# mcveanlab/Corticall

Measured on AMD Instinct MI355X. Metric: k-mers traversed/sec (whole node) + contigs/sec, k=47 3-color LdBG, higher is better.
Workload: dtype u64

## Files before the change

corticall_amd/csrc/capi.cpp:

```cpp
#include <string.h>

#include <memory>

#include "build.h"
#include "cursor.h"
#include "engine_host.h"
#include "linkbuild.h"
#include "mosaic.h"
#include "seeds.h"
#include "select.h"
#include "shard.h"
#include "sw.h"
#include "thread.h"
#include "unitigs.h"
#include "variants.h"

using namespace ldbg;

namespace ldbg {
int64_t sort_ctx_file(const std::string& in_path, const std::string& out_path, int device);
int64_t subset_ctx_file(const std::string& in_path, const int64_t* indices, int64_t n, const std::string& out_path);
int64_t join_ctx_files(const std::vector<std::string>& paths, const std::string& out_path, int device);
std::vector<uint8_t> join_ctx_image(const std::vector<std::string>& paths, int device, bool find_view);
void profile_reset_all();
// ... 786 lines not shown
}
ldbg_status ldbg_cursor_result_get(const ldbg_cursor_result* r, int64_t* offsets, uint64_t* kmer_words, int64_t* rec, int32_t* n_reverse, int32_t* n_forward,
                                   int64_t* seed_rec, uint8_t* end_reverse, uint8_t* end_forward, uint8_t* status) {
    return guard([&] { cursor_result_of(r).get(offsets, kmer_words, rec, n_reverse, n_forward, seed_rec, end_reverse, end_forward, status, false, nullptr); });
}
ldbg_status ldbg_cursor_result_get_dev(const ldbg_cursor_result* r, void* d_offsets, void* d_kmer_words, void* d_rec, void* d_n_reverse, void* d_n_forward,
                                       void* d_seed_rec, void* d_end_reverse, void* d_end_forward, void* d_status, void* stream) {
    return guard([&] {
        cursor_result_of(r).get(d_offsets, d_kmer_words, d_rec, d_n_reverse, d_n_forward, d_seed_rec, d_end_reverse, d_end_forward, d_status, true, (rt::stream_t)stream);
    });
}
ldbg_status ldbg_cursor_result_free(ldbg_cursor_result* r) { delete r; return LDBG_OK; }

static ldbg_status variant_batch_any(ldbg_engine* ce, ldbg_engine* pe, const char* seeds, int64_t n, bool on_device, int stop_colour, int64_t max_steps, uint64_t sum_mask,
                                     ldbg_variant_result** out) {
    return guard([&] {
        if (!ce || !pe || !out) throw StatusError(LDBG_ERR_ARG, "variant batch: null engine or result pointer");
        *out = nullptr;
        if (!ce->cursor_batch) ce->cursor_batch.reset(new CursorBatchHost(ce->e));
        if (!pe->cursor_batch) pe->cursor_batch.reset(new CursorBatchHost(pe->e));
        std::unique_ptr<VariantResult> r(variant_batch(ce->e, *ce->cursor_batch, pe->e, *pe->cursor_batch, seeds, n, on_device, stop_colour, max_steps, sum_mask));
        *out = new ldbg_variant_result{std::move(r)};
    });
}
ldbg_status ldbg_engine_variant_batch(ldbg_engine* child_engine, ldbg_engine* parent_engine, const char* seeds, int64_t n, int stop_colour, int64_t max_steps,
                                      uint64_t sum_mask, ldbg_variant_result** out) {
    return variant_batch_any(child_engine, parent_engine, seeds, n, false, stop_colour, max_steps, sum_mask, out);
}
ldbg_status ldbg_engine_variant_batch_device(ldbg_engine* child_engine, ldbg_engine* parent_engine, const void* d_seeds, int64_t n, int stop_colour, int64_t max_steps,
                                             uint64_t sum_mask, ldbg_variant_result** out) {
    return variant_batch_any(child_engine, parent_engine, (const char*)d_seeds, n, true, stop_colour, max_steps, sum_mask, out);
}
static const VariantResult& variant_result_of(const ldbg_variant_result* r) {
    if (!r || !r->r) throw StatusError(LDBG_ERR_ARG, "no variant result");
    return *r->r;
}
ldbg_status ldbg_variant_result_sizes(const ldbg_variant_result* r, int64_t* n_seeds, int* n_colours, int64_t* allele_bytes, int64_t* n_child_vertices,
                                      int64_t* n_parent_vertices, int* kmer_words) {
    return guard([&] {
        const VariantResult& v = variant_result_of(r);
        if (n_seeds) *n_seeds = v.n;
        if (n_colours) *n_colours = v.n_colours;
        if (allele_bytes) *allele_bytes = v.allele_bytes;
        if (n_child_vertices) *n_child_vertices = v.child ? v.child->total : 0;
        if (n_parent_vertices) *n_parent_vertices = v.parent ? v.parent->total : 0;
        if (kmer_words) *kmer_words = v.W;
    });
}
ldbg_status ldbg_variant_result_get(const ldbg_variant_result* r, const ldbg_variant_arrays* into) {
    return guard([&] {
        if (!into) throw StatusError(LDBG_ERR_ARG, "variant result: null arrays");
        variant_result_of(r).get(*into, false, nullptr);
    });
}
ldbg_status ldbg_variant_result_get_dev(const ldbg_variant_result* r, const ldbg_variant_arrays* into, void* stream) {
    return guard([&] {
        if (!into) throw StatusError(LDBG_ERR_ARG, "variant result: null arrays");
        variant_result_of(r).get(*into, true, (rt::stream_t)stream);
    });
}
ldbg_status ldbg_variant_result_free(ldbg_variant_result* r) { delete r; return LDBG_OK; }

ldbg_status ldbg_mosaic_align_batch(int device, const ldbg_mosaic_params* p, int64_t n, const char* queries, const int64_t* query_off, const int64_t* target_first,
                                    const char* targets, const int64_t* target_off, ldbg_mosaic_result** out) {
    return guard([&] {
        if (!out) throw StatusError(LDBG_ERR_ARG, "mosaic: null result pointer");
        *out = nullptr;
        if (!p) throw StatusError(LDBG_ERR_ARG, "mosaic: null parameters");
        std::unique_ptr<MosaicResult> r(mosaic_align_batch(device, *p, n, queries, query_off, target_first, targets, target_off));
        *out = new ldbg_mosaic_result{std::move(r)};
    });
}
static const MosaicResult& mosaic_result_of(const ldbg_mosaic_result* r) {
    if (!r || !r->r) throw StatusError(LDBG_ERR_ARG, "no mosaic result");
    return *r->r;
}
ldbg_status ldbg_mosaic_result_sizes(const ldbg_mosaic_result* r, int64_t* n, int64_t* path_entries) {
    return guard([&] {
        const MosaicResult& m = mosaic_result_of(r);
        if (n) *n = m.n;
        if (path_entries) *path_entries = m.path_off.back();
    });
}
ldbg_status ldbg_mosaic_result_get(const ldbg_mosaic_result* r, const ldbg_mosaic_arrays* into) {
    return guard([&] {
        if (!into) throw StatusError(LDBG_ERR_ARG, "mosaic result: null arrays");
        const MosaicResult& m = mosaic_result_of(r);
        auto copy = [](void* dst, const void* src, size_t bytes) { if (dst && bytes) memcpy(dst, src, bytes); };
        copy(into->status, m.status.data(), m.status.size());
        copy(into->llk, m.llk.data(), m.llk.size() * 8);
        copy(into->path_off, m.path_off.data(), m.path_off.size() * 8);
        copy(into->copy, m.copy.data(), m.copy.size() * 4);
        copy(into->state, m.state.data(), m.state.size() * 4);
        copy(into->pos, m.pos.data(), m.pos.size() * 4);
    });
}
ldbg_status ldbg_mosaic_result_free(ldbg_mosaic_result* r) { delete r; return LDBG_OK; }
ldbg_status ldbg_mosaic_tb_roundtrip(int device, double div, int64_t n, const int32_t* who, const int32_t* state, const int32_t* pos, int32_t* out) {
    return guard([&] { mosaic_tb_roundtrip(device, div, n, who, state, pos, out); });
}

ldbg_status ldbg_sw_align_batch(int device, int64_t n, const char* queries, const int64_t* query_off, const char* subjects, const int64_t* subject_off,
                                ldbg_sw_result** out) {
    return guard([&] {
        if (!out) throw StatusError(LDBG_ERR_ARG, "sw: null result pointer");
        *out = nullptr;
        std::unique_ptr<SwResult> r(sw_align_batch(device, n, queries, query_off, subjects, subject_off));
        *out = new ldbg_sw_result{std::move(r)};
    });
}
static const SwResult& sw_result_of(const ldbg_sw_result* r) {
    if (!r || !r->r) throw StatusError(LDBG_ERR_ARG, "no sw result");
    return *r->r;
}
ldbg_status ldbg_sw_result_sizes(const ldbg_sw_result* r, int64_t* n, int64_t* columns, int64_t* query_letters, int64_t* subject_letters) {
    return guard([&] {
        const SwResult& m = sw_result_of(r);
        if (n) *n = m.n;
        if (columns) *columns = m.col_off.back();
        if (query_letters) *query_letters = m.q_off.back();
        if (subject_letters) *subject_letters = m.s_off.back();
    });
}
ldbg_status ldbg_sw_result_get(const ldbg_sw_result* r, const ldbg_sw_arrays* into) {
    return guard([&] {
        if (!into) throw StatusError(LDBG_ERR_ARG, "sw result: null arrays");
        const SwResult& m = sw_result_of(r);
        auto copy = [](void* dst, const void* src, size_t bytes) { if (dst && bytes) memcpy(dst, src, bytes); };
        copy(into->status, m.status.data(), m.status.size());
        copy(into->score, m.score.data(), m.score.size() * 8);
        copy(into->end_q, m.end_q.data(), m.end_q.size() * 4);
        copy(into->end_s, m.end_s.data(), m.end_s.size() * 4);
        copy(into->begin_q, m.begin_q.data(), m.begin_q.size() * 4);
        copy(into->begin_s, m.begin_s.data(), m.begin_s.size() * 4);
        copy(into->aligned_len, m.aligned_len.data(), m.aligned_len.size() * 4);
        copy(into->edits, m.edits.data(), m.edits.size() * 4);
        copy(into->col_off, m.col_off.data(), m.col_off.size() * 8);
        copy(into->cols, m.cols.data(), m.cols.size());
        copy(into->q_off, m.q_off.data(), m.q_off.size() * 8);
        copy(into->q_letters, m.q_letters.data(), m.q_letters.size());
        copy(into->s_off, m.s_off.data(), m.s_off.size() * 8);
        copy(into->s_letters, m.s_letters.data(), m.s_letters.size());
    });
}
ldbg_status ldbg_sw_result_free(ldbg_sw_result* r) { delete r; return LDBG_OK; }

#ifdef LDBG_HOSTSIM
void ldbg_debug_ls(uint64_t* out) {
    auto& d = ldbg::ls_debug();
    out[0] = d.adds; out[1] = d.newkeys; out[2] = d.choices; out[3] = d.scan; out[4] = d.maxn; out[5] = d.steps; out[6] = d.sum_n;
    out[7] = d.runs_a; out[8] = d.runs_b; out[9] = d.run_vertices; out[10] = d.retries; out[11] = d.repeats;
    d = ldbg::LsDebug();
}
#endif
#ifdef LDBG_HOSTSIM
extern "C" void ldbg_hostsim_set_lanes(int n) { int v = 1; while (v * 2 <= n && v < 64) v *= 2; ::ldbg::sim::lanes_setting() = v; }
#endif
ldbg_status ldbg_profile_reset(void) { profile_reset_all(); return LDBG_OK; }
ldbg_status ldbg_profile_get(const char* family, double* total_ms, int64_t* launches) {
    profile_get(family, total_ms, launches);
    return LDBG_OK;
}

}
```

corticall_amd/csrc/engine.h:

```cpp
#pragma once
#include "graph.h"
#include "links.h"

namespace ldbg {

struct RunIndexView { const uint64_t* uinfo; const uint32_t* uo; const uint8_t* ubase; };

struct EngineView {
    GraphView g;
    uint32_t trav_mask, recruit_mask, join_mask;
    uint32_t trav_sel4, recruit_sel4;
    int first_trav;
    int stopper, max_len, connect_all, strict_flip;
    int lean_rows;
    int cursor_on;
    uint32_t link_flag_mask;
    LinksView links;
    RunIndexView runs;
};

enum : uint32_t {
    ST_OK = 0,
    ST_NULLPTR = 1,
    ST_LINKSTORE_FULL = 2,
    ST_BRANCH_NULL = 3,
    ST_COPY_OVERFLOW = 4,
    ST_POOL_FULL = 5,
    ST_STOPPER_CONFIG = 6,
    ST_DEPTH_OVERFLOW = 7,
    ST_TABLE_FULL = 8,
    ST_LOG_FULL = 9,
    ST_RETRY_PLAIN = 10,
    ST_MERGE_UNSUPPORTED = 11
};

LDBG_HOSTDEV uint64_t path_pack(int64_t idx, bool flip, unsigned base, int copy, bool quirk = false) {
    return (uint64_t)(idx + 1) | ((uint64_t)(flip ? 1 : 0) << 33) | ((uint64_t)(base & 3u) << 34) |
           (((uint64_t)(uint32_t)copy & 0xFFFFFFull) << 36) | ((uint64_t)(quirk ? 1 : 0) << 60);
}
LDBG_HOSTDEV bool path_quirk(uint64_t e) { return (e >> 60) & 1ull; }
LDBG_HOSTDEV int64_t path_idx(uint64_t e) { return (int64_t)(e & 0x1FFFFFFFFull) - 1; }
LDBG_HOSTDEV bool path_flip(uint64_t e) { return (e >> 33) & 1ull; }
LDBG_HOSTDEV unsigned path_base(uint64_t e) { return (unsigned)((e >> 34) & 3ull); }
LDBG_HOSTDEV int path_copy(uint64_t e) { int32_t v = (int32_t)((e >> 36) & 0xFFFFFFull); return (v << 8) >> 8; }

LDBG_HOSTDEV int popc4(uint32_t m) { return (int)((m & 1u) + ((m >> 1) & 1u) + ((m >> 2) & 1u) + ((m >> 3) & 1u)); }
LDBG_HOSTDEV unsigned lowbit4(uint32_t m) { return (m & 1u) ? 0u : ((m & 2u) ? 1u : ((m & 4u) ? 2u : 3u)); }

struct Node {
    int32_t idx;
    int32_t copy;
    uint32_t vslot;
    uint64_t vent;
    uint8_t flip;
    uint8_t fj;
    uint8_t npe;
    uint8_t lflags;
    uint8_t next_mask;
    uint8_t prev_mask;
    uint8_t base;
    uint8_t e1;
#ifdef LDBG_LEAN_PROFILE
    unsigned long long p1, p2;
#endif
    uint32_t ent1;
    uint64_t ui;
};

template <bool FEW = false>
LDBG_HOSTDEV void node_fill_bytes(const EngineView& e, Node& n, uint32_t edges4, const uint8_t* more, uint8_t fl) {
    const GraphView& g = e.g;
    n.npe = 0; n.fj = n.flip;
    n.lflags = fl & LDBG_ROW_LINK_BITS;
    if (e.strict_flip && (fl & LDBG_ROW_HASH_COLLISION)) n.fj = 0;
    const bool fj = n.fj != 0;
    uint32_t tb = edges4 & e.trav_sel4, rb = edges4 & e.recruit_sel4;
    tb |= tb >> 16; tb |= tb >> 8; rb |= rb >> 16; rb |= rb >> 8;
    if (!FEW)
        for (int col = 4; col < g.C; col++) {
            if ((e.trav_mask >> col) & 1u) tb |= more[col];
            if ((e.recruit_mask >> col) & 1u) rb |= more[col];
        }
    tb &= 0xffu; rb &= 0xffu;
    const uint32_t tfw = !fj ? tb & 0xf : tb >> 4, trn = !fj ? tb >> 4 : tb & 0xf;
    const uint32_t rfw = !fj ? rb & 0xf : rb >> 4, rrn = !fj ? rb >> 4 : rb & 0xf;
    const uint32_t tf = tfw, rf = rfw;
    const uint32_t tr = ((trn & 1u) << 3) | ((trn & 2u) << 1) | ((trn & 4u) >> 1) | ((trn & 8u) >> 3);
    const uint32_t rr = ((rrn & 1u) << 3) | ((rrn & 2u) << 1) | ((rrn & 4u) >> 1) | ((rrn & 8u) >> 3);
    n.next_mask = (uint8_t)(tf ? tf : rf);
    n.prev_mask = (uint8_t)(tr ? tr : rr);
}
LDBG_HOSTDEV void node_fill(const EngineView& e, Node& n) {
    const GraphView& g = e.g;
    n.ui = e.runs.uinfo && n.idx >= 0 ? e.runs.uinfo[n.idx] : 0ull;
    if (n.idx >= 0) {
        const uint8_t* row = graph_row(g, n.idx);
        const uint8_t* ed = row + g.edges_off;
        uint32_t edges4 = 0;
        for (int col = 0; col < g.C && col < 4; col++) edges4 |= (uint32_t)ed[col] << (8 * col);
        node_fill_bytes(e, n, edges4, ed, row[g.flags_off]);
    } else {
        n.npe = e.recruit_mask != 0 ? 1 : 0; n.lflags = 0; n.fj = n.flip;
        n.next_mask = n.prev_mask = 0;
    }
}

LDBG_HOSTDEV void node_child(const EngineView& e, const Node& p, bool fwd, unsigned base, Node& n) {
    const GraphView& g = e.g;
    const bool fj = p.fj != 0;
    const unsigned j = fwd ? (!fj ? base : 4u + (3u - base)) : (!fj ? 4u + base : (3u - base));
    const uint32_t ent = graph_nbr(g, p.idx, (int)j);
    n.idx = (int32_t)(ent & 0x7FFFFFFFu) - 1;
    n.copy = 0; n.vslot = 0; n.vent = 0; n.base = (uint8_t)base; n.e1 = 0; n.ent1 = 0;
    bool flip = (((ent >> 31) & 1u) != 0) != fj;
    if (n.idx >= 0 && (graph_row(g, n.idx)[g.flags_off] & LDBG_ROW_PALINDROME)) flip = false;
    n.flip = flip ? 1 : 0;
    node_fill(e, n);
}

template <int W>
LDBG_HOSTDEV Kmer<W> node_kmer(const EngineView& e, const Node& n) {
    Kmer<W> c = graph_key<W>(e.g, n.idx);
    return n.flip ? kmer_revcomp<W>(c, e.g.k) : c;
}
template <int W>
LDBG_HOSTDEV Kmer<W> node_o(const EngineView& e, const Node& n) {
    Kmer<W> c = graph_key<W>(e.g, n.idx);
    return n.fj ? kmer_revcomp<W>(c, e.g.k) : c;
}
template <int W>
LDBG_HOSTDEV Kmer<W> child_kmer(const EngineView& e, const Node& p, bool fwd, unsigned base) {
    Kmer<W> o = node_o<W>(e, p);
    return fwd ? kmer_next<W>(o, e.g.k, base) : kmer_prev<W>(o, e.g.k, base);
}
template <int W>
LDBG_HOSTDEV void node_find(const EngineView& e, const Kmer<W>& sk, Node& n) {
    bool fc;
    Kmer<W> c = kmer_canonical<W>(sk, e.g.k, &fc);
    n.idx = (int32_t)graph_find_canonical<W>(e.g, c);
    n.copy = 0; n.vslot = 0; n.vent = 0; n.base = 0; n.e1 = 0; n.ent1 = 0;
    n.flip = fc ? 1 : 0;
    node_fill(e, n);
    if (n.idx < 0 && e.strict_flip && fc)
        n.fj = kmer_java_hash<W>(c, e.g.k) != kmer_java_hash<W>(sk, e.g.k) ? 1 : 0;
}
LDBG_HOSTDEV void node_null(const EngineView& e, Node& n) {
    n.idx = -1; n.copy = 0; n.vslot = 0; n.vent = 0; n.e1 = 0; n.ent1 = 0; n.flip = 0; n.fj = 0; n.lflags = 0; n.base = 0;
    n.next_mask = n.prev_mask = 0; n.ui = 0;
    n.npe = e.recruit_mask != 0 ? 1 : 0;
}

struct VisitedTable {
    uint64_t* tab;
    uint32_t mask;
    uint32_t used;
};
#define LDBG_VT_KEY_MASK 0x3FFFFFFFFull
LDBG_HOSTDEV uint32_t vt_hash(uint64_t key) {
    uint32_t x = (uint32_t)key ^ ((uint32_t)(key >> 32) * 0x9E3779B1u);
    x ^= x >> 16; x *= 0x85EBCA6Bu; x ^= x >> 13; x *= 0xC2B2AE35u; x ^= x >> 16;
    return x;
}
LDBG_HOSTDEV uint64_t vt_key(int64_t idx, bool flip) { return ((uint64_t)(idx + 1) << 1) | (flip ? 1ull : 0ull); }
#ifdef LDBG_HOSTSIM
struct LsDebug { uint64_t adds = 0, newkeys = 0, choices = 0, scan = 0, maxn = 0, steps = 0, sum_n = 0, runs_a = 0, runs_b = 0, run_vertices = 0, retries = 0, repeats = 0; };
inline LsDebug& ls_debug() { static LsDebug d; return d; }
#endif
struct VtPeek { uint64_t e[4]; };
LDBG_HOSTDEV VtPeek vt_peek(const VisitedTable& t, uint32_t h) {
    VtPeek p;
#pragma unroll
    for (uint32_t q = 0; q < 4; q++) p.e[q] = LDBG_GLOBAL(const uint64_t, t.tab)[(h + q) & t.mask];
    return p;
}
LDBG_HOSTDEV uint32_t vt_probe_from(VisitedTable& t, uint64_t key, uint32_t h, VtPeek pk, uint64_t* ent) {
    while (true) {
#ifdef LDBG_HOSTSIM
        ls_debug().scan++;
#endif
        uint32_t q = 4;
        uint64_t ev = 0;
#pragma unroll
        for (int i = 3; i >= 0; i--) {
            const bool stop = pk.e[i] == 0 || (pk.e[i] & LDBG_VT_KEY_MASK) == key;
            q = stop ? (uint32_t)i : q;
            ev = stop ? pk.e[i] : ev;
        }
        if (q < 4) {
            const uint32_t slot = (h + q) & t.mask;
            if (ev == 0) { LDBG_GLOBAL(uint64_t, t.tab)[slot] = key; t.used++; ev = key; }
            *ent = ev;
            return slot;
        }
        h = (h + 4) & t.mask;
        pk = vt_peek(t, h);
    }
}
LDBG_HOSTDEV uint32_t vt_locate(VisitedTable& t, int64_t idx, bool flip, uint64_t* ent) {
    const uint64_t key = vt_key(idx, flip);
    const uint32_t h = vt_hash(key) & t.mask;
    return vt_probe_from(t, key, h, vt_peek(t, h), ent);
}
LDBG_HOSTDEV int vt_count_e(uint64_t e) { return (int)((e >> 48) & 0x7FFFull); }
#define LDBG_VT_EPOCH_MAX 0x3FFFu
LDBG_HOSTDEV bool vt_seen_e(uint64_t e, uint32_t epoch) { return (uint32_t)((e >> 34) & LDBG_VT_EPOCH_MAX) == epoch; }
LDBG_HOSTDEV uint64_t vt_with_seen(uint64_t e, uint32_t epoch) { return (e & ~((uint64_t)LDBG_VT_EPOCH_MAX << 34)) | ((uint64_t)epoch << 34); }
LDBG_HOSTDEV uint64_t vt_with_count(uint64_t e, int c) { return (e & ~(0x7FFFull << 48)) | ((uint64_t)(c & 0x7FFF) << 48); }
LDBG_HOSTDEV void node_locate(VisitedTable& t, Node& n) { if (n.idx >= 0) n.vslot = vt_locate(t, n.idx, n.flip != 0, &n.vent); }
LDBG_HOSTDEV int node_count(const Node& n) { return n.idx >= 0 ? vt_count_e(n.vent) : 0; }
LDBG_HOSTDEV void node_store(VisitedTable& t, Node& n, uint64_t val) { LDBG_GLOBAL(uint64_t, t.tab)[n.vslot] = val; n.vent = val; }
LDBG_HOSTDEV void node_sync(Node& n, const Node& written) { if (n.idx >= 0 && written.idx >= 0 && n.vslot == written.vslot) n.vent = written.vent; }
LDBG_HOSTDEV uint32_t node_child_entry(const EngineView& e, const Node& p, bool fwd, unsigned base) {
    const bool fj = p.fj != 0;
    const unsigned j = fwd ? (!fj ? base : 4u + (3u - base)) : (!fj ? 4u + base : (3u - base));
    return graph_nbr(e.g, p.idx, (int)j);
}
LDBG_HOSTDEV unsigned nbr_slot(bool fj, bool fwd, unsigned base) {
    return fwd ? (!fj ? base : 4u + (3u - base)) : (!fj ? 4u + base : (3u - base));
}
LDBG_HOSTDEV uint32_t nbr_pick(const uint32_t (&nb)[8], unsigned j) {
    uint32_t v = reg_opaque(nb[0]);
#pragma unroll
    for (unsigned q = 1; q < 8; q++) v = j == q ? reg_opaque(nb[q]) : v;
    return v;
}
LDBG_HOSTDEV bool row_is_packed(const GraphView& g) { return g.C <= 3 && (g.edges_off & 3) == 0 && (g.nbr_off & 15) == 0 && (g.stride & 15) == 0; }
LDBG_HOSTDEV constexpr bool row_layout_is_packed(int W, int C) {
    return C <= 3 && (row_layout(W, C).edges_off & 3) == 0 && (row_layout(W, C).nbr_off & 15) == 0 && (row_layout(W, C).stride & 15) == 0;
}
template <bool LEAN = false>
LDBG_HOSTDEV void node_from_entry(const EngineView& e, VisitedTable& t, const Node& p, uint32_t ent, unsigned base, bool fwd, Node& n) {
    const GraphView& g = e.g;
    const bool fj = p.fj != 0;
    n.idx = (int32_t)(ent & 0x7FFFFFFFu) - 1;
    n.copy = 0; n.vslot = 0; n.vent = 0; n.base = (uint8_t)base; n.e1 = 0; n.ent1 = 0;
    bool flip = (((ent >> 31) & 1u) != 0) != fj;
    const bool rec = LEAN || n.idx >= 0;
    const bool early = LEAN || (rec && (g.k & 1));
    uint64_t key = 0;
    VtPeek e0 = {{0, 0, 0, 0}};
    uint32_t h = 0;
    if (early) { key = vt_key(n.idx, flip); h = vt_hash(key) & t.mask; e0 = vt_peek(t, h); }
    uint32_t nb[8] = {0, 0, 0, 0, 0, 0, 0, 0};
    uint32_t ef = 0;
    const bool packed = LEAN || row_is_packed(g);
    uint64_t ui = 0;
    if (rec && e.runs.uinfo) ui = LDBG_GLOBAL(const uint64_t, e.runs.uinfo)[n.idx];
    if (rec) {
        const uint8_t* row = graph_row(g, n.idx);
        if (packed) {
            struct alignas(16) U4 { uint32_t x, y, z, w; };
            const U4 a = *(const U4*)(row + g.nbr_off), b = *(const U4*)(row + g.nbr_off + 16);
            ef = *(const uint32_t*)(row + g.edges_off);
            nb[0] = a.x; nb[1] = a.y; nb[2] = a.z; nb[3] = a.w; nb[4] = b.x; nb[5] = b.y; nb[6] = b.z; nb[7] = b.w;
        } else {
            const uint32_t* nbp = (const uint32_t*)(row + g.nbr_off);
#pragma unroll
            for (int q = 0; q < 8; q++) nb[q] = nbp[q];
        }
    }
    if (!LEAN && rec && !(g.k & 1) && (graph_row(g, n.idx)[g.flags_off] & LDBG_ROW_PALINDROME)) flip = false;
#ifdef LDBG_LEAN_PROFILE
    if (LEAN) {
        asm volatile("" ::: "memory");
        const unsigned long long t1 = __builtin_readcyclecounter();
        asm volatile("s_waitcnt vmcnt(0)" ::: "memory");
        const unsigned long long t2 = __builtin_readcyclecounter();
        n.p1 = t1; n.p2 = t2;
    }
#endif
    n.flip = flip ? 1 : 0;
    if (LEAN) node_fill_bytes<true>(e, n, ef & ((1u << (8 * g.C)) - 1u), nullptr, (uint8_t)(ef >> (8 * g.C)));
    else if (rec && packed) node_fill_bytes(e, n, ef & ((1u << (8 * g.C)) - 1u), nullptr, (uint8_t)(ef >> (8 * g.C)));
    else node_fill(e, n);
    n.ui = ui;
    if (rec) {
        const uint32_t m = fwd ? n.next_mask : n.prev_mask;
        const unsigned j = nbr_slot(n.fj != 0, fwd, lowbit4(m));
        const uint32_t v = nbr_pick(nb, j);
        const bool one = popc4(m) == 1;
        n.ent1 = one ? v : 0u; n.e1 = one ? 1 : 0;
        if (!early) { key = vt_key(n.idx, flip); h = vt_hash(key) & t.mask; e0 = vt_peek(t, h); }
        n.vslot = vt_probe_from(t, key, h, e0, &n.vent);
    }
}
struct NodeLoad {
    uint32_t nb[8];
    uint32_t ef, h;
    uint64_t ui, key;
    VtPeek e0;
    int32_t idx;
    bool flip;
};
LDBG_HOSTDEV void node_issue_lean(const EngineView& e, const VisitedTable& t, bool parent_fj, uint32_t ent, NodeLoad& L) {
    const GraphView& g = e.g;
    L.idx = (int32_t)(ent & 0x7FFFFFFFu) - 1;
    L.flip = (((ent >> 31) & 1u) != 0) != parent_fj;
    L.key = vt_key(L.idx, L.flip);
    L.h = vt_hash(L.key) & t.mask;
    L.e0 = vt_peek(t, L.h);
    L.ui = e.runs.uinfo ? LDBG_GLOBAL(const uint64_t, e.runs.uinfo)[L.idx] : 0ull;
    const uint8_t* row = graph_row(g, L.idx);
    struct alignas(16) U4 { uint32_t x, y, z, w; };
    const U4 a = *(const U4*)(row + g.nbr_off), b = *(const U4*)(row + g.nbr_off + 16);
    L.ef = *(const uint32_t*)(row + g.edges_off);
    L.nb[0] = a.x; L.nb[1] = a.y; L.nb[2] = a.z; L.nb[3] = a.w; L.nb[4] = b.x; L.nb[5] = b.y; L.nb[6] = b.z; L.nb[7] = b.w;
}
LDBG_HOSTDEV bool vt_round_covers(const VisitedTable& t, uint32_t h, uint32_t slot) { return slot != 0xFFFFFFFFu && ((slot - h) & t.mask) < 4u; }
LDBG_HOSTDEV void node_finish_lean(const EngineView& e, VisitedTable& t, const NodeLoad& L, unsigned base, bool fwd, Node& n, uint32_t claimed0 = 0xFFFFFFFFu,
                                   uint32_t claimed1 = 0xFFFFFFFFu) {
    const GraphView& g = e.g;
    n.idx = L.idx;
    n.copy = 0; n.vslot = 0; n.vent = 0; n.base = (uint8_t)base; n.e1 = 0; n.ent1 = 0;
    n.flip = L.flip ? 1 : 0;
    node_fill_bytes<true>(e, n, L.ef & ((1u << (8 * g.C)) - 1u), nullptr, (uint8_t)(L.ef >> (8 * g.C)));
    n.ui = L.ui;
    const uint32_t m = fwd ? n.next_mask : n.prev_mask;
    const unsigned j = nbr_slot(n.fj != 0, fwd, lowbit4(m));
    const uint32_t v = nbr_pick(L.nb, j);
    const bool one = popc4(m) == 1;
    n.ent1 = one ? v : 0u; n.e1 = one ? 1 : 0;
    const bool stale = vt_round_covers(t, L.h, claimed0) || vt_round_covers(t, L.h, claimed1);
    n.vslot = vt_probe_from(t, L.key, L.h, stale ? vt_peek(t, L.h) : L.e0, &n.vent);
}
LDBG_HOSTDEV void node_child_located(const EngineView& e, VisitedTable& t, const Node& p, bool fwd, unsigned base, Node& n) {
    node_from_entry(e, t, p, node_child_entry(e, p, fwd, base), base, fwd, n);
}

struct LsElem {
    uint32_t str_off;
    uint32_t birth;
    int32_t hash;
    uint32_t key_seq;
    uint16_t len;
    uint16_t pos;
    uint8_t comp;
    uint8_t nxn;
    uint16_t nx;
};
static_assert(sizeof(LsElem) == 24, "LsElem is moved as six words");
#ifdef LDBG_HOSTSIM
struct LdsShadow { const char* base = nullptr; size_t bytes = 0; std::vector<uint8_t> written; bool on = false; };
inline LdsShadow& lds_shadow() { static LdsShadow s; return s; }
inline void lds_shadow_begin(const void* base, size_t bytes) {
    LdsShadow& s = lds_shadow();
    static const bool want = getenv("LDBG_HOSTSIM_LDS_CHECK") != nullptr;
    s.on = want;
    if (!want) return;
    s.base = (const char*)base; s.bytes = bytes; s.written.assign(bytes / 24 + 1, 0);
}
inline void lds_shadow_touch(const void* q, bool write) {
    LdsShadow& s = lds_shadow();
    if (!s.on || (const char*)q < s.base || (const char*)q >= s.base + s.bytes) return;
    const size_t i = (size_t)((const char*)q - s.base) / 24;
    if (write) { s.written[i] = 1; return; }
    if (!s.written[i]) {
        fprintf(stderr, "[hostsim] link-store element %zu of the simulated LDS is read before this wavefront wrote it\n", i);
        void* bt[48]; const int nb = backtrace(bt, 48); backtrace_symbols_fd(bt, nb, 2);
        abort();
    }
}
#endif
template <typename P> LDBG_HOSTDEV LsElem ls_elem_in(P q) {
#ifdef LDBG_HOSTSIM
    lds_shadow_touch((const void*)q, false);
#endif
    uint32_t w[6];
#pragma unroll
    for (int i = 0; i < 6; i++) w[i] = q[i];
    LsElem x;
    __builtin_memcpy(&x, w, 24);
    return x;
}
template <typename P> LDBG_HOSTDEV void ls_elem_out(P q, const LsElem& x) {
#ifdef LDBG_HOSTSIM
    lds_shadow_touch((const void*)q, true);
#endif
    uint32_t w[6];
    __builtin_memcpy(w, &x, 24);
#pragma unroll
    for (int i = 0; i < 6; i++) q[i] = w[i];
}
#ifdef LDBG_HOSTSIM
inline uint32_t& ls_peak_elements() { static uint32_t p = 0; return p; }
#define LDBG_LS_PEAK(i) do { if ((uint32_t)(i) + 1u > ::ldbg::ls_peak_elements()) ::ldbg::ls_peak_elements() = (uint32_t)(i) + 1u; } while (0)
#else
#define LDBG_LS_PEAK(i) ((void)0)
#endif
#if defined(LDBG_WALK_DIAG) && defined(__HIP_DEVICE_COMPILE__)
#define LDBG_LS_COUNT(ctr, tail) do { if (ctr) { atomicAdd((ctr), 1ull); if (tail) atomicAdd((ctr) + 1, 1ull); } } while (0)
#else
#define LDBG_LS_COUNT(ctr, tail) ((void)0)
#endif
struct LinkStoreDev {
#ifdef LDBG_WALK_DIAG
    unsigned long long* diag;
#endif
    LsElem* fast;
    LsElem* el;
    uint32_t fast_cap, fast_stride;
    uint32_t cap;
    uint32_t n;
    uint32_t java_cap;
    uint32_t nkeys;
    uint32_t next_seq;
    uint32_t age;
    uint32_t n_new;
    bool overflow;
};
LDBG_HOSTDEV LsElem ls_get(const LinkStoreDev& s, uint32_t i) {
    LDBG_LS_COUNT(s.diag, i >= s.fast_cap);
    if (i < s.fast_cap) return ls_elem_in(LDBG_LDS(const uint32_t, s.fast + i * s.fast_stride));
    return ls_elem_in(LDBG_GLOBAL(const uint32_t, s.el + (i - s.fast_cap)));
}
LDBG_HOSTDEV void ls_set(LinkStoreDev& s, uint32_t i, const LsElem& x) {
    LDBG_LS_COUNT(s.diag, i >= s.fast_cap);
    LDBG_LS_PEAK(i);
    if (i < s.fast_cap) ls_elem_out(LDBG_LDS(uint32_t, s.fast + i * s.fast_stride), x);
    else ls_elem_out(LDBG_GLOBAL(uint32_t, s.el + (i - s.fast_cap)), x);
}
LDBG_HOSTDEV void ls_clear(LinkStoreDev& s) { s.n = 0; s.java_cap = 0; s.nkeys = 0; s.next_seq = 0; s.age = 0; s.n_new = 0; s.overflow = false; }
struct LsSaved { uint32_t n, java_cap, nkeys, next_seq, age, n_new; uint8_t overflow; };
LDBG_HOSTDEV LsSaved ls_save(const LinkStoreDev& s) { return LsSaved{s.n, s.java_cap, s.nkeys, s.next_seq, s.age, s.n_new, (uint8_t)(s.overflow ? 1 : 0)}; }
LDBG_HOSTDEV void ls_restore(LinkStoreDev& s, const LsSaved& v) {
    s.n = v.n; s.java_cap = v.java_cap; s.nkeys = v.nkeys; s.next_seq = v.next_seq; s.age = v.age; s.n_new = v.n_new; s.overflow = v.overflow != 0;
}
struct LsWave {
#ifdef LDBG_WALK_DIAG
    unsigned long long* diag;
#endif
    LsElem* fast;
    uint32_t stride;
    uint32_t fast_cap;
    LsElem* el;
    uint32_t ecap;
};
LDBG_HOSTDEV unsigned ls_char(const LinksView& L, const LsElem& x, uint32_t i) {
    unsigned b = L.bases[x.str_off + i];
    return x.comp ? 3u - b : b;
}
LDBG_HOSTDEV void ls_fill_nx(const LinksView& L, LsElem& x) {
    uint32_t nx = 0, cnt = 0;
    for (uint32_t i = 0; i < 8; i++) {
        if ((uint32_t)x.pos + i >= x.len) break;
        nx |= (uint32_t)ls_char(L, x, (uint32_t)x.pos + i) << (2 * i);
        cnt++;
    }
    x.nx = (uint16_t)nx; x.nxn = (uint8_t)cnt;
}
LDBG_HOSTDEV void ls_first_nx(const JuncRec& jr, LsElem& x) {
    const uint32_t cnt = jr.len < 8u ? jr.len : 8u;
    const uint32_t mask = (1u << (2 * cnt)) - 1u;
    const uint32_t nx = jr.is_fw >> 16;
    x.nx = (uint16_t)((x.comp ? ~nx : nx) & mask);
    x.nxn = (uint8_t)cnt;
}
LDBG_HOSTDEV unsigned ls_cur(const LsElem& x) { return x.nx & 3u; }
LDBG_HOSTDEV void ls_advance(const LinksView& L, LsElem& x) {
    x.pos++;
    x.nx >>= 2; x.nxn--;
    if (x.nxn == 0) ls_fill_nx(L, x);
}
LDBG_HOSTDEV bool ls_same_string(const LinksView& L, const LsElem& a, const LsElem& b) {
    if (a.str_off == b.str_off && a.comp == b.comp) return true;
    if (a.len != b.len || a.hash != b.hash) return false;
    for (uint32_t i = 0; i < a.len; i++) if (ls_char(L, a, i) != ls_char(L, b, i)) return false;
    return true;
}
LDBG_HOSTDEV bool ls_key_alive(const LinkStoreDev& s, uint32_t key_seq, uint32_t n) {
    for (uint32_t i = n; i-- > 0;) if (ls_get(s, i).key_seq == key_seq) return true;
    return false;
}
LDBG_HOSTDEV void ls_add(const LinksView& L, LinkStoreDev& s, uint32_t jlo, uint32_t jhi, bool query_flipped, bool fwd) {
    for (uint32_t j = jlo; j < jhi; j++) {
        const JuncRec jr = L.junc[j];
        bool lgf = ((jr.is_fw & 1u) != 0) != query_flipped;
// ... 184 lines not shown
```

corticall_amd/csrc/runstep.h:

```cpp
#pragma once
#include "lscoop.h"
#include "runs.h"
#include "strand.h"

namespace ldbg {

#define LDBG_RUN_MIN 8u

struct Piece {
    uint32_t S, E;
    uint32_t q, n;
    bool plus, asc;
};
LDBG_DEV void piece_cut(uint32_t& S, uint32_t& E, uint32_t pos, uint32_t cut) {
    if (cut >= S && cut <= E) {
        if (pos < cut) E = cut - 1u;
        else if (pos > cut) S = cut + 1u;
        else S = E = pos;
    }
}
LDBG_DEV Piece piece_make(uint64_t ui, bool flip, bool fwd, uint32_t S, uint32_t E) {
    Piece p;
    const uint32_t pos = ui_pos(ui);
    p.S = S; p.E = E;
    p.plus = flip == ui_orient(ui);
    p.asc = p.plus == fwd;
    p.q = p.asc ? pos - p.S : p.E - pos;
    p.n = p.E - p.S + 1u;
    return p;
}
LDBG_DEV Piece piece_of(uint64_t ui, bool flip, bool fwd, uint32_t seed_pos) {
    const uint32_t pos = ui_pos(ui);
    uint32_t S = pos - ui_dstart(ui), E = pos + ui_dend(ui);
    piece_cut(S, E, pos, seed_pos);
    return piece_make(ui, flip, fwd, S, E);
}
LDBG_DEV uint64_t piece_key(uint32_t S, bool plus) { return (1ull << 33) | ((uint64_t)S << 1) | (plus ? 1ull : 0ull); }
LDBG_DEV uint64_t piece_key(const Piece& p) { return piece_key(p.S, p.plus); }

struct RunState {
    uint32_t seed_pos;
    uint32_t seen_marks;
    uint32_t choices;
    uint32_t anchor_at;
    uint32_t anchor_gv, anchor_marks, anchor_n, anchor_cap;
    uint32_t period;
    uint64_t anchor_sig;
    uint64_t anchor_cv, anchor_t;
};

struct WalkLane { StrandState st; RunState rs; };
using StrandSave = LaneSave<WalkLane>;

#define LDBG_SNAP_CAP 64u
#define LDBG_REPEAT_FROM 4u
struct LsSnap { uint32_t str_off, pos_comp, age, key_seq; };
LDBG_DEV uint64_t sig_mix(uint64_t x) { x ^= x >> 30; x *= 0xBF58476D1CE4E5B9ull; x ^= x >> 27; x *= 0x94D049BB133111EBull; x ^= x >> 31; return x; }
LDBG_DEV uint64_t node_key(const Node& n) { return n.idx >= 0 ? vt_key(n.idx, n.flip != 0) : 0ull; }
LDBG_DEV uint64_t walk_signature(const StrandState& st, const LinkStoreDev& ls) {
    uint64_t h = sig_mix(node_key(st.cv) ^ (node_key(st.cu.nxt) << 30) ^ ((uint64_t)ls.n << 50) ^ ((uint64_t)ls.java_cap << 40));
    for (uint32_t i = 0; i < ls.n; i++) {
        const LsElem x = ls_get(ls, i);
        h = sig_mix(h ^ (uint64_t)x.str_off ^ ((uint64_t)x.pos << 32) ^ ((uint64_t)x.comp << 48));
        h = sig_mix(h ^ (uint64_t)(ls.age - x.birth));
    }
    return h;
}
LDBG_DEV void walk_snapshot(const StrandState& st, const LinkStoreDev& ls, LsSnap* snap) {
    for (uint32_t i = 0; i < ls.n; i++) {
        const LsElem x = ls_get(ls, i);
        LsSnap v;
        v.str_off = x.str_off; v.pos_comp = (uint32_t)x.pos | ((uint32_t)x.comp << 16); v.age = ls.age - x.birth; v.key_seq = x.key_seq;
        LDBG_GLOBAL(LsSnap, snap)[i] = v;
    }
}
LDBG_DEV bool walk_same_store(const LinkStoreDev& ls, const LsSnap* snap) {
    for (uint32_t i = 0; i < ls.n; i++) {
        const LsElem x = ls_get(ls, i);
        const LsSnap v = LDBG_GLOBAL(const LsSnap, snap)[i];
        if (v.str_off != x.str_off || v.pos_comp != ((uint32_t)x.pos | ((uint32_t)x.comp << 16)) || v.age != ls.age - x.birth) return false;
        for (uint32_t j = 0; j < i; j++) {
            const uint32_t kj = ls_get(ls, j).key_seq, sj = LDBG_GLOBAL(const LsSnap, snap)[j].key_seq;
            const int now = x.key_seq < kj ? -1 : (x.key_seq > kj ? 1 : 0), then = v.key_seq < sj ? -1 : (v.key_seq > sj ? 1 : 0);
            if (now != then) return false;
        }
    }
    return true;
}
LDBG_DEV bool periodic_check(const WalkArgs& a, StrandState& st, const LinkStoreDev& ls, RunState& rs, LsSnap* snap) {
    rs.choices++;
    if (rs.choices < LDBG_REPEAT_FROM || ls.n > LDBG_SNAP_CAP || !st.cu.has || st.cv.idx < 0 || st.cu.nxt.idx < 0) return false;
    if (st.cv.copy == 0) return false;
    const uint64_t sig = walk_signature(st, ls);
    const bool live = rs.anchor_at != 0u && rs.seen_marks == rs.anchor_marks;
    if (live && sig == rs.anchor_sig && ls.n == rs.anchor_n && ls.java_cap == rs.anchor_cap && node_key(st.cv) == rs.anchor_cv && node_key(st.cu.nxt) == rs.anchor_t &&
        st.gV > rs.anchor_gv && walk_same_store(ls, snap)) {
        const uint32_t P = st.gV - rs.anchor_gv;
        if (rs.period == P && st.gV >= 2u * P && st.gV <= (uint32_t)a.e.max_len) {
            const uint32_t R = (uint32_t)a.e.max_len + 1u - st.gV;
            if (!path_append_pair(a, st.s, st.pw, pd_repeat_head(R), (uint64_t)(st.gV - 2u * P) | ((uint64_t)P << 32))) { st.status = ST_POOL_FULL; return true; }
            st.gV += R; st.iters += R + 1u;
#ifdef LDBG_HOSTSIM
            ls_debug().repeats++;
#endif
            return true;
        }
        rs.period = P;
        rs.anchor_gv = st.gV; rs.anchor_at = rs.choices;
        return false;
    }
    if (!live || rs.choices >= 2u * rs.anchor_at) {
        rs.anchor_at = rs.choices; rs.anchor_gv = st.gV; rs.anchor_marks = rs.seen_marks; rs.anchor_n = ls.n; rs.anchor_cap = ls.java_cap; rs.period = 0u;
        rs.anchor_sig = sig; rs.anchor_cv = node_key(st.cv); rs.anchor_t = node_key(st.cu.nxt);
        walk_snapshot(st, ls, snap);
    }
    return false;
}

LDBG_DEV bool run_entry_a(const EngineView& e, const StrandState& st, const RunState& rs) {
    const Node& cv = st.cv;
    const Node& t = st.cu.nxt;
    if (!ui_valid(cv.ui) || !ui_valid(t.ui)) return false;
    const Piece pc = piece_of(cv.ui, cv.flip != 0, st.fwd, rs.seed_pos);
    if (pc.q != 0u || pc.n < LDBG_RUN_MIN) return false;
    const Piece pt = piece_of(t.ui, t.flip != 0, st.fwd, rs.seed_pos);
    return pt.S == pc.S && pt.E == pc.E && pt.plus == pc.plus && pt.q == 1u;
}
LDBG_DEV bool run_mode_a(const WalkArgs& a, const StrandState& st, const RunState& rs) {
    return lean_cursor_ok(a.e, st) && st.gV >= 2u && st.gV <= (uint32_t)a.e.max_len && run_entry_a(a.e, st, rs);
}
LDBG_DEV bool run_b_vertex(const EngineView& e, const StrandState& st) {
    const Node& cv = st.cv;
    if (st.status != ST_OK || (e.cursor_on && st.cu.has) || !(e.g.k & 1)) return false;
    if (cv.idx < 0 || cv.npe || cv.flip != cv.fj || !ui_valid(cv.ui)) return false;
    const int acopy = cv.copy < 0 ? -cv.copy : cv.copy;
    return acopy >= vt_count_e(cv.vent) && acopy + 1 <= 32767;
}
LDBG_DEV bool run_mode_b(const WalkArgs& a, const StrandState& st, const RunState& rs) {
    if (!run_b_vertex(a.e, st) || st.gV < 1u) return false;
    const Piece pc = piece_of(st.cv.ui, st.cv.flip != 0, st.fwd, rs.seed_pos);
    return pc.q == 1u && pc.n >= LDBG_RUN_MIN;
}

LDBG_DEV void run_vertex(const EngineView& e, VisitedTable& vt, uint32_t pos, bool inv, bool fwd, Node& n) {
    const uint32_t u = LDBG_GLOBAL(const uint32_t, e.runs.uo)[pos];
    const unsigned bb = LDBG_GLOBAL(const uint8_t, e.runs.ubase)[pos];
    const unsigned first = !inv ? (bb & 3u) : 3u - ((bb >> 2) & 3u), last = !inv ? ((bb >> 2) & 3u) : 3u - (bb & 3u);
    Node parent;
    parent.fj = 0;
    const uint32_t ent = ((u & 0x7FFFFFFFu) + 1u) | ((((u >> 31) != 0u) != inv) ? 0x80000000u : 0u);
    node_from_entry(e, vt, parent, ent, fwd ? last : first, fwd, n);
}

LDBG_DEV bool run_emit(const WalkArgs& a, StrandState& st, uint32_t len, uint32_t acopy, const Piece& pc, uint32_t hi) {
    if (len == 0u) return true;
    const uint32_t first = pc.asc ? pc.S + 2u : pc.E - 2u;
    return path_append_pair(a, st.s, st.pw, pd_run_head(len, acopy, pc.asc, !pc.plus), (uint64_t)first | ((uint64_t)hi << 32));
}

template <int W>
LDBG_DEV bool run_step(const WalkArgs& a, StrandState& st, LinkStoreDev& ls, RunState& rs, bool mode_a) {
    const EngineView& e = a.e;
    const bool fwd = st.fwd;
    Node& cv = st.cv;
    const Piece pc = piece_of(cv.ui, cv.flip != 0, fwd, rs.seed_pos);
    const uint32_t n = pc.n, nB = n - 4u;
    const bool inv = !pc.plus;
    Node y, z;
    const uint32_t used0 = st.vt.used;
    uint64_t eB = 0;
    const uint64_t kB = piece_key(pc);
    const uint32_t hB = vt_hash(kB) & st.vt.mask;
    uint32_t slotB;
    if (e.lean_rows) {
        const uint32_t py = pc.asc ? pc.E - 1u : pc.S + 1u, pz = pc.asc ? pc.E : pc.S;
        const uint32_t uy = LDBG_GLOBAL(const uint32_t, e.runs.uo)[py], uz = LDBG_GLOBAL(const uint32_t, e.runs.uo)[pz];
        const unsigned by = LDBG_GLOBAL(const uint8_t, e.runs.ubase)[py], bz = LDBG_GLOBAL(const uint8_t, e.runs.ubase)[pz];
        const VtPeek pB = vt_peek(st.vt, hB);
        NodeLoad ly, lz;
        node_issue_lean(e, st.vt, false, ((uy & 0x7FFFFFFFu) + 1u) | ((((uy >> 31) != 0u) != inv) ? 0x80000000u : 0u), ly);
        node_issue_lean(e, st.vt, false, ((uz & 0x7FFFFFFFu) + 1u) | ((((uz >> 31) != 0u) != inv) ? 0x80000000u : 0u), lz);
        auto travel_base = [&](unsigned bb) { const unsigned first = !inv ? (bb & 3u) : 3u - ((bb >> 2) & 3u), last = !inv ? ((bb >> 2) & 3u) : 3u - (bb & 3u); return fwd ? last : first; };
        uint32_t u0 = st.vt.used;
        node_finish_lean(e, st.vt, ly, travel_base(by), fwd, y);
        const uint32_t cy = st.vt.used != u0 ? y.vslot : 0xFFFFFFFFu;
        u0 = st.vt.used;
        node_finish_lean(e, st.vt, lz, travel_base(bz), fwd, z, cy);
        const uint32_t cz = st.vt.used != u0 ? z.vslot : 0xFFFFFFFFu;
        const bool staleB = vt_round_covers(st.vt, hB, cy) || vt_round_covers(st.vt, hB, cz);
        slotB = vt_probe_from(st.vt, kB, hB, staleB ? vt_peek(st.vt, hB) : pB, &eB);
    } else {
        run_vertex(e, st.vt, pc.asc ? pc.E - 1u : pc.S + 1u, inv, fwd, y);
        run_vertex(e, st.vt, pc.asc ? pc.E : pc.S, inv, fwd, z);
        slotB = vt_probe_from(st.vt, kB, hB, vt_peek(st.vt, hB), &eB);
    }
    rs.seen_marks += st.vt.used - used0;
    const int cntB = vt_count_e(eB), cntY = vt_count_e(y.vent);
    const int64_t allowed = (int64_t)e.max_len - (int64_t)st.gV + 1;
    if (mode_a) {
        Node& t = st.cu.nxt;
        const uint32_t ep = st.cu.epoch;
        const int cntT = vt_count_e(t.vent);
        const bool seenB = vt_seen_e(eB, ep), seenY = vt_seen_e(y.vent, ep), seenZ = vt_seen_e(z.vent, ep);
        const uint32_t steps = n - 2u;
        const bool full = allowed >= (int64_t)steps;
        const uint32_t k = full ? steps : (uint32_t)allowed;
        bool odd = false;
        if (ls.n == 0u) odd = seenB || (seenY && k >= n - 3u);
        odd = odd || (k >= 2u && cntT + 1 > 32767) || (k >= 3u && cntB + 1 > 32767);
        if (odd) {
#ifdef LDBG_HOSTSIM
            ls_debug().retries++;
#endif
            st.status = ST_RETRY_PLAIN; return true;
        }
#ifdef LDBG_HOSTSIM
        ls_debug().runs_a++; ls_debug().run_vertices += k;
#endif
        if (ls_num_new(ls) > 0) ls_increment_ages(ls);
        st.iters += k;
        const int acv = cv.copy < 0 ? -cv.copy : cv.copy;
        Node tv = t;
        tv.copy = fwd ? cntT : -cntT;
        bool ok = path_append(a, st.s, st.pw, pack_vertex(tv));
        ok = ok && run_emit(a, st, k - 1u < nB ? k - 1u : nB, (uint32_t)cntB, pc, 0u);
        if (!full) {
            if (!ok) { st.status = ST_POOL_FULL; return true; }
            st.gV += k; st.iters += 1u;
            return true;
        }
        y.copy = fwd ? cntY : -cntY;
        ok = ok && path_append(a, st.s, st.pw, pack_vertex(y));
        if (!ok) { st.status = ST_POOL_FULL; return true; }
        st.gV += k;
        node_store(st.vt, cv, vt_with_count(cv.vent, acv + 1));
        node_store(st.vt, t, vt_with_count(t.vent, cntT + 1));
        uint64_t nb = vt_with_count(eB, cntB + 1);
        if (!seenB) { nb = vt_with_seen(nb, ep); rs.seen_marks++; }
        LDBG_GLOBAL(uint64_t, st.vt.tab)[slotB] = nb;
        if (!seenY) { node_store(st.vt, y, vt_with_seen(y.vent, ep)); rs.seen_marks++; }
        if (!seenZ) { node_store(st.vt, z, vt_with_seen(z.vent, ep)); rs.seen_marks++; }
        st.cu.has = !seenZ || ls.n > 0u;
        if (st.cu.has) st.cu.nxt = z;
        cv = y;
        st.cu.cur = cv;
        return false;
    }
    const uint32_t want = n - 3u;
    uint32_t by_counts = want;
    if (cntB > 0) by_counts = 0u;
    else if (cntY > 0) by_counts = n - 4u;
    uint32_t k = by_counts;
    if (allowed < (int64_t)k) k = allowed > 0 ? (uint32_t)allowed : 0u;
    const bool ended = k < want;
#ifdef LDBG_HOSTSIM
    ls_debug().runs_b++; ls_debug().run_vertices += k;
#endif
    st.iters += k + (ended ? 1u : 0u);
    bool ok = run_emit(a, st, k < nB ? k : nB, 0u, pc, 0u);
    if (k == want) { y.copy = 0; ok = ok && path_append(a, st.s, st.pw, pack_vertex(y)); }
    if (!ok) { st.status = ST_POOL_FULL; return true; }
    st.gV += k;
    if (ended) return true;
    const int acv = cv.copy < 0 ? -cv.copy : cv.copy;
    node_store(st.vt, cv, vt_with_count(cv.vent, acv + 1));
    LDBG_GLOBAL(uint64_t, st.vt.tab)[slotB] = vt_with_count(eB, 1);
    cv = y;
    return false;
}

}
```

Before: 201.3 billion.

## Trim lean run-step node loads by deriving neighbor and unitig info

The lean run step stops loading the per-node unitig info word and instead rebuilds it from the current vertex's run info and position. It loads only the half of the neighbor row the traversal direction needs, and skips the neighbor load for y by deriving its successor from z's run entry. It also pre-scans B's visited-table peek so the common non-stale case skips a re-scan, and recomputes hashes in finish instead of carrying them in registers. This cuts global memory traffic and register pressure, at the cost of extra ALU work and the assumption that derived values match the stored ones, which is checked only under the host simulator.

```diff
diff --git a/corticall_amd/csrc/capi.cpp b/corticall_amd/csrc/capi.cpp
--- a/corticall_amd/csrc/capi.cpp
+++ b/corticall_amd/csrc/capi.cpp
@@ -962,6 +962,11 @@
     out[7] = d.runs_a; out[8] = d.runs_b; out[9] = d.run_vertices; out[10] = d.retries; out[11] = d.repeats;
     d = ldbg::LsDebug();
 }
+void ldbg_debug_run_reads(uint64_t* out) {
+    auto& d = ldbg::ls_debug();
+    out[0] = d.stale_rounds; out[1] = d.derived; out[2] = d.derived_bad;
+    d.stale_rounds = d.derived = d.derived_bad = 0;
+}
 #endif
 #ifdef LDBG_HOSTSIM
 extern "C" void ldbg_hostsim_set_lanes(int n) { int v = 1; while (v * 2 <= n && v < 64) v *= 2; ::ldbg::sim::lanes_setting() = v; }
diff --git a/corticall_amd/csrc/engine.h b/corticall_amd/csrc/engine.h
--- a/corticall_amd/csrc/engine.h
+++ b/corticall_amd/csrc/engine.h
@@ -163,7 +163,8 @@
 }
 LDBG_HOSTDEV uint64_t vt_key(int64_t idx, bool flip) { return ((uint64_t)(idx + 1) << 1) | (flip ? 1ull : 0ull); }
 #ifdef LDBG_HOSTSIM
-struct LsDebug { uint64_t adds = 0, newkeys = 0, choices = 0, scan = 0, maxn = 0, steps = 0, sum_n = 0, runs_a = 0, runs_b = 0, run_vertices = 0, retries = 0, repeats = 0; };
+struct LsDebug { uint64_t adds = 0, newkeys = 0, choices = 0, scan = 0, maxn = 0, steps = 0, sum_n = 0, runs_a = 0, runs_b = 0, run_vertices = 0, retries = 0, repeats = 0;
+                 uint64_t stale_rounds = 0, derived = 0, derived_bad = 0; };
 inline LsDebug& ls_debug() { static LsDebug d; return d; }
 #endif
 struct VtPeek { uint64_t e[4]; };
@@ -285,43 +286,85 @@
     }
 }
 struct NodeLoad {
-    uint32_t nb[8];
-    uint32_t ef, h;
-    uint64_t ui, key;
+    uint32_t nb[4];
+    uint32_t ef;
     VtPeek e0;
     int32_t idx;
     bool flip;
 };
-LDBG_HOSTDEV void node_issue_lean(const EngineView& e, const VisitedTable& t, bool parent_fj, uint32_t ent, NodeLoad& L) {
+template <bool NBR = true>
+LDBG_HOSTDEV void node_issue_lean(const EngineView& e, const VisitedTable& t, bool parent_fj, uint32_t ent, bool fwd, NodeLoad& L) {
     const GraphView& g = e.g;
     L.idx = (int32_t)(ent & 0x7FFFFFFFu) - 1;
     L.flip = (((ent >> 31) & 1u) != 0) != parent_fj;
-    L.key = vt_key(L.idx, L.flip);
-    L.h = vt_hash(L.key) & t.mask;
-    L.e0 = vt_peek(t, L.h);
-    L.ui = e.runs.uinfo ? LDBG_GLOBAL(const uint64_t, e.runs.uinfo)[L.idx] : 0ull;
+    L.e0 = vt_peek(t, vt_hash(vt_key(L.idx, L.flip)) & t.mask);
     const uint8_t* row = graph_row(g, L.idx);
-    struct alignas(16) U4 { uint32_t x, y, z, w; };
-    const U4 a = *(const U4*)(row + g.nbr_off), b = *(const U4*)(row + g.nbr_off + 16);
     L.ef = *(const uint32_t*)(row + g.edges_off);
-    L.nb[0] = a.x; L.nb[1] = a.y; L.nb[2] = a.z; L.nb[3] = a.w; L.nb[4] = b.x; L.nb[5] = b.y; L.nb[6] = b.z; L.nb[7] = b.w;
+    L.nb[0] = L.nb[1] = L.nb[2] = L.nb[3] = 0u;
+    if (NBR) {
+        struct alignas(16) U4 { uint32_t x, y, z, w; };
+        const U4 a = *(const U4*)(row + g.nbr_off + (fwd != L.flip ? 0 : 16));
+        L.nb[0] = a.x; L.nb[1] = a.y; L.nb[2] = a.z; L.nb[3] = a.w;
+    }
 }
 LDBG_HOSTDEV bool vt_round_covers(const VisitedTable& t, uint32_t h, uint32_t slot) { return slot != 0xFFFFFFFFu && ((slot - h) & t.mask) < 4u; }
-LDBG_HOSTDEV void node_finish_lean(const EngineView& e, VisitedTable& t, const NodeLoad& L, unsigned base, bool fwd, Node& n, uint32_t claimed0 = 0xFFFFFFFFu,
-                                   uint32_t claimed1 = 0xFFFFFFFFu) {
+struct VtHit { uint32_t q; uint64_t ev; };
+LDBG_HOSTDEV VtHit vt_round_scan(const VtPeek& pk, uint64_t key) {
+    VtHit r;
+    r.q = 4; r.ev = 0;
+#pragma unroll
+    for (int i = 3; i >= 0; i--) {
+        const bool stop = pk.e[i] == 0 || (pk.e[i] & LDBG_VT_KEY_MASK) == key;
+        r.q = stop ? (uint32_t)i : r.q;
+        r.ev = stop ? pk.e[i] : r.ev;
+    }
+    return r;
+}
+LDBG_HOSTDEV uint32_t vt_probe_hit(VisitedTable& t, uint64_t key, uint32_t h, VtHit hit, uint64_t* ent) {
+#ifdef LDBG_HOSTSIM
+    ls_debug().scan++;
+#endif
+    if (hit.q < 4) {
+        const uint32_t slot = (h + hit.q) & t.mask;
+        uint64_t ev = hit.ev;
+        if (ev == 0) { LDBG_GLOBAL(uint64_t, t.tab)[slot] = key; t.used++; ev = key; }
+        *ent = ev;
+        return slot;
+    }
+    h = (h + 4) & t.mask;
+    return vt_probe_from(t, key, h, vt_peek(t, h), ent);
+}
+template <bool NBR = true>
+LDBG_HOSTDEV void node_finish_lean(const EngineView& e, VisitedTable& t, const NodeLoad& L, uint64_t ui, unsigned base, bool fwd, Node& n, uint32_t claimed0 = 0xFFFFFFFFu,
+                                   uint32_t claimed1 = 0xFFFFFFFFu, uint32_t ent1 = 0u) {
     const GraphView& g = e.g;
-    n.idx = L.idx;
+    n.idx = (int32_t)reg_opaque((uint32_t)L.idx);
     n.copy = 0; n.vslot = 0; n.vent = 0; n.base = (uint8_t)base; n.e1 = 0; n.ent1 = 0;
     n.flip = L.flip ? 1 : 0;
     node_fill_bytes<true>(e, n, L.ef & ((1u << (8 * g.C)) - 1u), nullptr, (uint8_t)(L.ef >> (8 * g.C)));
-    n.ui = L.ui;
+    n.ui = ui;
     const uint32_t m = fwd ? n.next_mask : n.prev_mask;
     const unsigned j = nbr_slot(n.fj != 0, fwd, lowbit4(m));
-    const uint32_t v = nbr_pick(L.nb, j);
+    uint32_t v = ent1;
+    if (NBR) {
+        v = reg_opaque(L.nb[0]);
+#pragma unroll
+        for (unsigned q = 1; q < 4; q++) v = (j & 3u) == q ? reg_opaque(L.nb[q]) : v;
+    }
+    if (n.fj != n.flip) v = graph_nbr(g, n.idx, (int)j);
     const bool one = popc4(m) == 1;
+#ifdef LDBG_HOSTSIM
+    ls_debug().derived++;
+    if ((one && v != graph_nbr(g, n.idx, (int)j)) || ui != (e.runs.uinfo ? e.runs.uinfo[n.idx] : 0ull)) ls_debug().derived_bad++;
+#endif
     n.ent1 = one ? v : 0u; n.e1 = one ? 1 : 0;
-    const bool stale = vt_round_covers(t, L.h, claimed0) || vt_round_covers(t, L.h, claimed1);
-    n.vslot = vt_probe_from(t, L.key, L.h, stale ? vt_peek(t, L.h) : L.e0, &n.vent);
+    const uint64_t key = vt_key(n.idx, L.flip);
+    const uint32_t h = vt_hash(key) & t.mask;
+    const bool stale = vt_round_covers(t, h, claimed0) || vt_round_covers(t, h, claimed1);
+#ifdef LDBG_HOSTSIM
+    if (stale) ls_debug().stale_rounds++;
+#endif
+    n.vslot = vt_probe_from(t, key, h, stale ? vt_peek(t, h) : L.e0, &n.vent);
 }
 LDBG_HOSTDEV void node_child_located(const EngineView& e, VisitedTable& t, const Node& p, bool fwd, unsigned base, Node& n) {
     node_from_entry(e, t, p, node_child_entry(e, p, fwd, base), base, fwd, n);
diff --git a/corticall_amd/csrc/runstep.h b/corticall_amd/csrc/runstep.h
--- a/corticall_amd/csrc/runstep.h
+++ b/corticall_amd/csrc/runstep.h
@@ -150,6 +150,11 @@
     parent.fj = 0;
     const uint32_t ent = ((u & 0x7FFFFFFFu) + 1u) | ((((u >> 31) != 0u) != inv) ? 0x80000000u : 0u);
     node_from_entry(e, vt, parent, ent, fwd ? last : first, fwd, n);
+}
+
+LDBG_DEV uint64_t run_ui(uint64_t at, uint32_t pos, uint32_t u) {
+    const uint32_t S0 = ui_pos(at) - ui_dstart(at), E0 = ui_pos(at) + ui_dend(at);
+    return ui_pack(pos, pos - S0, E0 - pos, (u >> 31) != 0u);
 }
 
 LDBG_DEV bool run_emit(const WalkArgs& a, StrandState& st, uint32_t len, uint32_t acopy, const Piece& pc, uint32_t hi) {
@@ -173,22 +178,28 @@
     const uint32_t hB = vt_hash(kB) & st.vt.mask;
     uint32_t slotB;
     if (e.lean_rows) {
+        const VtPeek pB = vt_peek(st.vt, hB);
         const uint32_t py = pc.asc ? pc.E - 1u : pc.S + 1u, pz = pc.asc ? pc.E : pc.S;
         const uint32_t uy = LDBG_GLOBAL(const uint32_t, e.runs.uo)[py], uz = LDBG_GLOBAL(const uint32_t, e.runs.uo)[pz];
         const unsigned by = LDBG_GLOBAL(const uint8_t, e.runs.ubase)[py], bz = LDBG_GLOBAL(const uint8_t, e.runs.ubase)[pz];
-        const VtPeek pB = vt_peek(st.vt, hB);
+        const VtHit hitB = vt_round_scan(pB, kB);
+        const uint32_t ey = ((uy & 0x7FFFFFFFu) + 1u) | ((((uy >> 31) != 0u) != inv) ? 0x80000000u : 0u);
+        const uint32_t ez = ((uz & 0x7FFFFFFFu) + 1u) | ((((uz >> 31) != 0u) != inv) ? 0x80000000u : 0u);
         NodeLoad ly, lz;
-        node_issue_lean(e, st.vt, false, ((uy & 0x7FFFFFFFu) + 1u) | ((((uy >> 31) != 0u) != inv) ? 0x80000000u : 0u), ly);
-        node_issue_lean(e, st.vt, false, ((uz & 0x7FFFFFFFu) + 1u) | ((((uz >> 31) != 0u) != inv) ? 0x80000000u : 0u), lz);
+        node_issue_lean<false>(e, st.vt, false, ey, fwd, ly);
+        node_issue_lean(e, st.vt, false, ez, fwd, lz);
         auto travel_base = [&](unsigned bb) { const unsigned first = !inv ? (bb & 3u) : 3u - ((bb >> 2) & 3u), last = !inv ? ((bb >> 2) & 3u) : 3u - (bb & 3u); return fwd ? last : first; };
         uint32_t u0 = st.vt.used;
-        node_finish_lean(e, st.vt, ly, travel_base(by), fwd, y);
+        node_finish_lean<false>(e, st.vt, ly, run_ui(cv.ui, py, uy), travel_base(by), fwd, y, 0xFFFFFFFFu, 0xFFFFFFFFu, (ez & 0x7FFFFFFFu) | ((ey ^ ez) & 0x80000000u));
         const uint32_t cy = st.vt.used != u0 ? y.vslot : 0xFFFFFFFFu;
         u0 = st.vt.used;
-        node_finish_lean(e, st.vt, lz, travel_base(bz), fwd, z, cy);
+        node_finish_lean(e, st.vt, lz, run_ui(cv.ui, pz, uz), travel_base(bz), fwd, z, cy);
         const uint32_t cz = st.vt.used != u0 ? z.vslot : 0xFFFFFFFFu;
         const bool staleB = vt_round_covers(st.vt, hB, cy) || vt_round_covers(st.vt, hB, cz);
-        slotB = vt_probe_from(st.vt, kB, hB, staleB ? vt_peek(st.vt, hB) : pB, &eB);
+#ifdef LDBG_HOSTSIM
+        if (staleB) ls_debug().stale_rounds++;
+#endif
+        slotB = staleB ? vt_probe_from(st.vt, kB, hB, vt_peek(st.vt, hB), &eB) : vt_probe_hit(st.vt, kB, hB, hitB, &eB);
     } else {
         run_vertex(e, st.vt, pc.asc ? pc.E - 1u : pc.S + 1u, inv, fwd, y);
         run_vertex(e, st.vt, pc.asc ? pc.E : pc.S, inv, fwd, z);
```

Result: no change. 202.8 billion (median of 6 runs) (+0.7%).
